# madsjulia/GeostatInversion.jl

Hardware: AMD Instinct MI355X
Metric: randSVD GB/s + top-k singular-value rel-err, n=1e6 rank=256 (higher is better)
Workload: dtype f64

## Files before the change

geostatinversion.jl_amd/csrc/api.cpp:

```cpp
#include <cmath>
#include <cstdlib>
#include <cstring>
#include <memory>
#include <new>
#include <string>
#include <vector>
#include "../../include/gsi_hip.h"
#include "pcga.hpp"
#include "pointcov.hpp"
#include "fftrf_points.hpp"
#include "cg_state.hpp"

using namespace gsi;

struct gsi_ctx {
  Context c;
};
struct gsi_op {
  Operator op;
};
struct gsi_mat {
  gsi_ctx* ctx;
  Buf buf;
  int64_t rows, cols;
// ... 1149 lines not shown
    Backend* be = ctx->c.be.get();
    Buf Wd(be, (size_t)n * l), V(be, (size_t)n * l), S(be, (size_t)l);
    be->upload2d(Wd.p, n, W, n, n, l);
    svd_tall(ctx->c, Wd.p, n, l, -1, V.p, S.p);
    be->download2d(V_out, n, V.p, n, n, l);
    be->download2d(S_out, l, S.p, l, l, 1);
    check_async_errors(ctx->c);
  });
}

int gsi_gemm(gsi_ctx* ctx, int trans, int64_t m, int64_t l, int64_t k, double alpha, const double* A,
             int64_t lda, const double* B, int64_t ldb, double* C, int64_t ldc) {
  return guarded([&] {
    REQUIRE(ctx && A && B && C, "NULL argument");
    REQUIRE(m >= 1 && l >= 1 && k >= 1, "bad shape");
    const int64_t ar = trans ? k : m, ac = trans ? m : k;
    REQUIRE(lda >= ar && ldb >= k && ldc >= m, "leading dimension too small");
    Backend* be = ctx->c.be.get();
    Buf Ad(be, (size_t)ar * ac), Bd(be, (size_t)k * l), Cd(be, (size_t)m * l);
    be->upload2d(Ad.p, ar, A, lda, ar, ac);
    be->upload2d(Bd.p, k, B, ldb, k, l);
    if (trans) be->gemm_tn(m, l, k, alpha, Ad.p, ar, Bd.p, k, 0.0, Cd.p, m);
    else be->gemm_nn(m, l, k, alpha, Ad.p, ar, Bd.p, k, 0.0, Cd.p, m);
    be->download2d(C, ldc, Cd.p, m, m, l);
    check_async_errors(ctx->c);
  });
}

int gsi_gemm_view(gsi_ctx* ctx, int form, int trans, int64_t m, int64_t l, int64_t k, double alpha, double beta,
                  const double* A, int64_t lda, int64_t a_off, const double* B, int64_t ldb, int64_t b_off, double* C,
                  int64_t ldc, int64_t c_off, int64_t m_full, int64_t r0, int64_t* plan_out) {
  return guarded([&] {
    REQUIRE(ctx && A && C && plan_out, "NULL argument");
    REQUIRE(form >= 0 && form <= 3, "gemm_view: form is 0 (gemm), 1 (syrk upper), 2 (trmm upper) or 3 (NN row block)");
    REQUIRE(m >= 1 && l >= 1 && k >= 1, "bad shape");
    REQUIRE(form == 1 || B, "NULL argument");
    REQUIRE(form == 0 || (alpha == 1.0 && beta == 0.0), "gemm_view: forms 1 to 3 compute C = op(A) B (alpha 1, beta 0)");
    REQUIRE(form == 0 || !trans, "gemm_view: trans belongs to form 0");
    REQUIRE(form != 1 || m == l, "gemm_view: form 1 is the l x l product A'A (m == l)");
    REQUIRE(form != 3 || (r0 >= 0 && r0 + m <= m_full), "gemm_view: row block outside the full product");
    const bool tn = trans || form == 1;
    const int64_t ar = (form == 3) ? m_full : (tn ? k : m), ac = tn ? m : k;
    const int64_t crows = (form == 3) ? m_full : m;
    REQUIRE(lda >= ar && ldc >= crows && (form == 1 || ldb >= k), "leading dimension too small");
    REQUIRE(a_off >= 0 && b_off >= 0 && c_off >= 0, "negative offset");
    Backend* be = ctx->c.be.get();
    const size_t na = (size_t)a_off + (size_t)lda * (size_t)ac, nc = (size_t)c_off + (size_t)ldc * (size_t)l;
    const size_t nb = (form == 1) ? 1 : (size_t)b_off + (size_t)ldb * (size_t)l;
    Buf Ad(be, na), Bd(be, nb), Cd(be, nc);
    be->fill_bytes(Ad.p, 0xFF, na);
    be->fill_bytes(Bd.p, 0xFF, nb);
    be->upload2d(Ad.p + a_off, lda, A, ar, ar, ac);
    if (form != 1) be->upload2d(Bd.p + b_off, ldb, B, k, k, l);
    be->upload2d(Cd.p, (int64_t)nc, C, (int64_t)nc, (int64_t)nc, 1);
    be->gemm_view(form, trans != 0, m, l, k, alpha, Ad.p + a_off, lda, Bd.p + b_off, ldb, beta, Cd.p + c_off, ldc, m_full, r0,
                  plan_out);
    be->download2d(C, (int64_t)nc, Cd.p, (int64_t)nc, (int64_t)nc, 1);
    check_async_errors(ctx->c);
  });
}

int gsi_cq_gram_round(gsi_ctx* ctx, int64_t l, int check, const double* gram, double* R, double* X, int32_t* flag_out,
                      int32_t* series_out, double* norm_out) {
  return guarded([&] {
    REQUIRE(ctx && gram && R && X && flag_out && series_out && norm_out, "NULL argument");
    REQUIRE(l >= 1 && l <= 384, "cq_gram_round: 1 <= l <= 384");
    Backend* be = ctx->c.be.get();
    Buf Gd(be, (size_t)l * l), Xd(be, (size_t)l * l);
    be->fill_bytes(Xd.p, 0xFF, (size_t)l * l);
    be->upload2d(Gd.p, l, gram, l, l, l);
    int32_t out2[2] = {0, 0};
    be->cq_gram_round_view(Gd.p, l, Xd.p, check != 0, out2, norm_out);
    be->download2d(R, l, Gd.p, l, l, l);
// ... 665 lines not shown
```

geostatinversion.jl_amd/csrc/backend.hpp:

```cpp
#pragma once
#include <cstddef>
#include <cstdint>
#include <stdexcept>
#include <string>

namespace gsi {

struct Error : std::runtime_error {
  int code;
  Error(int c, const std::string& msg) : std::runtime_error(msg), code(c) {}
};

enum Phase : int {
  PH_GEMM_N = 0, PH_GEMM_T = 1, PH_LU = 2, PH_QR = 3, PH_SVD = 4, PH_SMALL_GEMM = 5,
  PH_COMM = 6, PH_OTHER = 7, PH_COMM_WAIT = 8, PH_COUNT = 9
};

struct FwdProduct {
  int64_t nobs = 0, n = 0, nnz = 0, nseg = 0, maxlen = 0;
  const int64_t* segptr = nullptr;
  const int64_t* rowseg = nullptr;
  const int32_t* colidx = nullptr;
  const double* vals = nullptr;
  const double* w = nullptr;
// ... 20 lines not shown

  virtual double* alloc(size_t count) = 0;
  virtual void release(double* p) = 0;
  virtual int64_t bytes_in_use() const = 0;
  virtual void release_cache() {}
  virtual void upload2d(double* dst, int64_t ldd, const double* host, int64_t ldh, int64_t rows, int64_t cols) = 0;
  virtual void download2d(double* host, int64_t ldh, const double* src, int64_t lds, int64_t rows, int64_t cols) = 0;
  virtual void copy2d(double* dst, int64_t ldd, const double* src, int64_t lds, int64_t rows, int64_t cols) = 0;
  virtual void fill_zero(double* p, size_t count) = 0;
  virtual void sync() = 0;
  virtual int64_t upload_block_rows(int64_t rows, int64_t cols) { (void)cols; return rows; }
  virtual void* upload2d_begin(double* dst, int64_t ldd, const double* host, int64_t ldh, int64_t rows, int64_t cols,
                               int64_t block_rows) {
    (void)block_rows;
    upload2d(dst, ldd, host, ldh, rows, cols);
    return nullptr;
  }
  virtual void pinned_copy_rate(int64_t bytes, double* h2d_gbs, double* d2h_gbs) { (void)bytes; *h2d_gbs = 0.0; *d2h_gbs = 0.0; }
  virtual void upload2d_wait_block(void* handle, int64_t b) { (void)handle; (void)b; }
  virtual void upload2d_end(void* handle) { (void)handle; }

  virtual void gemm_nn(int64_t m, int64_t l, int64_t k, double alpha, const double* A, int64_t lda,
                       const double* B, int64_t ldb, double beta, double* C, int64_t ldc) = 0;
  virtual void gemm_nn_rowblock(int64_t m_full, int64_t r0, int64_t mb, int64_t l, int64_t k, const double* A, int64_t lda,
                                const double* B, int64_t ldb, double* C, int64_t ldc) {
    (void)m_full;
    gemm_nn(mb, l, k, 1.0, A + r0, lda, B, ldb, 0.0, C + r0, ldc);
  }
  virtual void gemm_tn(int64_t m, int64_t l, int64_t k, double alpha, const double* A, int64_t lda,
                       const double* B, int64_t ldb, double beta, double* C, int64_t ldc) = 0;

  virtual void gemm_view(int form, bool trans, int64_t m, int64_t l, int64_t k, double alpha, const double* A, int64_t lda,
                         const double* B, int64_t ldb, double beta, double* C, int64_t ldc, int64_t m_full, int64_t r0,
                         int64_t* plan8) {
    (void)form; (void)trans; (void)m; (void)l; (void)k; (void)alpha; (void)A; (void)lda; (void)B; (void)ldb; (void)beta;
    (void)C; (void)ldc; (void)m_full; (void)r0; (void)plan8;
    throw Error(1 , "gemm_view: not available on this backend");
  }
  virtual void fill_bytes(double* p, int byte, size_t count) {
    (void)p; (void)byte; (void)count;
    throw Error(1 , "fill_bytes: not available on this backend");
  }

  virtual void gemm_nn_gridcov(int64_t m, int64_t l, int64_t k, const double* tab, int64_t nx, int64_t ny,
                               int64_t roff, int64_t koff, const double* B, int64_t ldb, double* C,
                               int64_t ldc) = 0;

  virtual void gemm_nn_pointcov(int64_t m, int64_t l, int64_t k, const double* pts, int d, int kind, double ell,
                                double sigma2, double nugget, int64_t roff, int64_t koff, const double* B, int64_t ldb,
                                double* C, int64_t ldc) = 0;

  virtual void* fftcov_create(const int64_t N[3], double beta, int fftrf) = 0;
  virtual void* fftcov_create_lags(const int64_t N[3], int kind, const double ell[3], double theta, double sigma2,
                                   double nugget, const double* table, const double* table_mirror) {
    (void)N; (void)kind; (void)ell; (void)theta; (void)sigma2; (void)nugget; (void)table; (void)table_mirror;
    throw Error(1 , "fft covariance from a covariance function or table: not supported by this backend");
  }
  virtual void fftcov_destroy(void* plan) = 0;
  virtual void fftcov_apply(void* plan, int64_t l, const double* X, int64_t ldx, double* Y, int64_t ldy) = 0;

  virtual void lu_L(double* Y, int64_t m, int64_t l, int64_t ld, int32_t* ipiv_host_or_null) = 0;
  virtual bool lu_L_keep(double* Y, int64_t m, int64_t l, int64_t ld, int32_t** ipiv_dev) {
    (void)Y; (void)m; (void)l; (void)ld; (void)ipiv_dev;
    return false;
  }
  virtual int lus_block() const = 0;
  virtual void lus_u12_leaf(const double* Yloc, int64_t ld, int64_t row0, int64_t jb, int64_t j0, int w, double* U12) = 0;
  virtual void lus_pending(double* Yloc, int64_t mloc, int64_t ld, int64_t row0, int64_t jb, int64_t j0, int w,
                           const double* U12) = 0;
// ... 293 lines not shown
```

geostatinversion.jl_amd/csrc/gemm_f64.hip:

```cpp
#include <hip/hip_runtime.h>
#include <cstdint>
#include <cstdlib>
#include <type_traits>
#include <algorithm>
#include "hip_common.hpp"
#include "pointcov.hpp"
#include "pointcov_gen.hpp"

namespace gsi { namespace hipk {

#define GSI_GEMM_TILE_COUNTERS_32 1
#include "gemm_f64_kernel.inc.hpp"
void gemm_dispatch_gen1(int nt, dim3 grid, hipStream_t st, int64_t M, int64_t L, int64_t K, const double* A, int64_t lda,
                        const double* B, int64_t ldb, double* C, int64_t ldc, double alpha, double beta, double* slabs,
                        int64_t kchunk, int nchunks_x, int wide, int xmode, int tri, const GenA& gen, int64_t nitems);

__global__ void splitk_reduce_kernel(int64_t M, int64_t L, int nsplit, const double* __restrict__ slabs,
                                     double* __restrict__ C, int64_t ldc, double alpha, double beta) {
  const int64_t total = M * L;
  for (int64_t idx = (int64_t)blockIdx.x * blockDim.x + threadIdx.x; idx < total;
       idx += (int64_t)gridDim.x * blockDim.x) {
    double s = 0.0;
    for (int sp = 0; sp < nsplit; ++sp) s += slabs[(int64_t)sp * total + idx];
    const int64_t r = idx % M, c = idx / M;
// ... 53 lines not shown
  if (M <= 0 || L <= 0) return max_grid <= 0;
  const uint64_t lim = (uint64_t)1 << 32;
  const uint64_t bspan = 8ull * ((uint64_t)(NTMAX * 16) * (uint64_t)ldb + BK);
  const uint64_t aspan = (gen != nullptr) ? 0ull : 8ull * ((uint64_t)(transA ? BMT : BK) * (uint64_t)lda + BMT);
  const bool big = bspan >= lim || aspan >= lim;
  const int64_t tiles = (L + 15) / 16;
  const int ntmax = gemm_chunk_tiles(tri);
  const int64_t nchunks = (tiles + ntmax - 1) / ntmax;
  const int nt = (int)((tiles + nchunks - 1) / nchunks);
  const int64_t rowblocks = (M + BMT - 1) / BMT;
  int64_t active = rowblocks * nchunks;
  if (tri == 1) {
    active = 0;
    for (int64_t rb = 0; rb < rowblocks; ++rb)
      for (int64_t cb = 0; cb < nchunks; ++cb)
        if (cb >= (rb * BMT) / ((int64_t)nt * 16)) ++active;
  }
  const int nsplit = (force_nsplit > 0) ? force_nsplit : ((K > 0) ? gemm_choose_split(active, K) : 1);
  int64_t kchunk = (K + nsplit - 1) / nsplit;
  kchunk = ((kchunk + BK - 1) / BK) * BK;
  if (kchunk == 0) kchunk = BK;
  const int ns_eff = (K > 0) ? (int)((K + kchunk - 1) / kchunk) : 1;
  dim3 grid((unsigned)active, (unsigned)ns_eff, 1);
  double* slabs = (ns_eff > 1) ? ws : nullptr;
  static const int ncus = [] { int dev = 0, n = 256; hipDeviceProp_t pr; if (hipGetDevice(&dev) == hipSuccess && hipGetDeviceProperties(&pr, dev) == hipSuccess) n = pr.multiProcessorCount; return n; }();
  static const bool persist_on = !(getenv("GSI_GEMM_PERSIST") != nullptr && getenv("GSI_GEMM_PERSIST")[0] == '0');
  int64_t nitems = 0;
  const bool a_ok = ((uintptr_t)A & 15) == 0 && (lda & 1) == 0;
  const bool b_ok = ((uintptr_t)B & 15) == 0 && (ldb & 1) == 0;
  const bool irregular_x = a_ok && (!b_ok || L % ((int64_t)nt * 16) != 0);
  const int wide = a_ok ? 1 : 0;
  const int xmode = big ? 2 : (irregular_x ? 1 : 0);
  if (persist_on && gen == nullptr && xmode == 0 && tri == 0 && ns_eff == 1 && (ncus & 7) == 0 && active >= 2 * (int64_t)ncus &&
      K <= 128 * BK) {
    nitems = active;
    grid.x = (unsigned)((max_grid > 0 && max_grid < ncus) ? max_grid : ncus);
  }
  if (max_grid > 0 && nitems == 0 && ((int64_t)grid.x * (int64_t)grid.y > (int64_t)max_grid || ns_eff != 1)) return false;
  if (plan != nullptr) *plan = {nt, nchunks, xmode, wide, ns_eff, nitems > 0 ? 1 : 0, (int64_t)grid.x, active};
  if (query_only) return true;
  const GenA none = {nullptr, 1, 0, 0, 0, 0.0, 0.0, 0.0};
  if (gen != nullptr && gen_mode == 2)
    launch_dispatch<false, 2>(nt, grid, st, M, L, K, A, lda, B, ldb, C, ldc, alpha, beta, slabs, kchunk, (int)nchunks, wide, xmode, tri, *gen, nitems);
  else if (gen != nullptr)
    gemm_dispatch_gen1(nt, grid, st, M, L, K, A, lda, B, ldb, C, ldc, alpha, beta, slabs, kchunk, (int)nchunks, wide, xmode, tri, *gen, nitems);
  else if (transA)
    launch_dispatch<true, 0>(nt, grid, st, M, L, K, A, lda, B, ldb, C, ldc, alpha, beta, slabs, kchunk, (int)nchunks, wide, xmode, tri, none, nitems);
  else
    launch_dispatch<false, 0>(nt, grid, st, M, L, K, A, lda, B, ldb, C, ldc, alpha, beta, slabs, kchunk, (int)nchunks, wide, xmode, tri, none, nitems);
  if (ns_eff > 1) {
    const int64_t total = M * L;
    int blocks = (int)((total + 255) / 256);
    if (blocks > 2048) blocks = 2048;
    hipLaunchKernelGGL(splitk_reduce_kernel, dim3(blocks), dim3(256), 0, st, M, L, ns_eff, slabs, C, ldc,
                       alpha, beta);
  }
  return true;
}

void gemm_splitk_reduce(hipStream_t st, int64_t M, int64_t L, int nsplit, const double* slabs, double* C, int64_t ldc) {
  const int64_t total = M * L;
  int blocks = (int)((total + 255) / 256);
  if (blocks > 2048) blocks = 2048;
  hipLaunchKernelGGL(splitk_reduce_kernel, dim3(blocks), dim3(256), 0, st, M, L, nsplit, slabs, C, ldc, 1.0, 0.0);
}

void gemm_f64(hipStream_t st, bool transA, int64_t M, int64_t L, int64_t K, double alpha, const double* A,
              int64_t lda, const double* B, int64_t ldb, double beta, double* C, int64_t ldc, double* ws, GemmPlan* plan) {
  gemm_launch(st, transA, nullptr, M, L, K, alpha, A, lda, B, ldb, beta, C, ldc, ws, 0, 1, 0, plan);
}

bool gemm_f64_nn_capped(hipStream_t st, int64_t M, int64_t L, int64_t K, const double* A, int64_t lda, const double* B,
                        int64_t ldb, double* C, int64_t ldc, int max_grid, bool query_only, GemmPlan* plan) {
  if (max_grid < 8 || (max_grid & 7) != 0) return false;
  return gemm_launch(st, false, nullptr, M, L, K, 1.0, A, lda, B, ldb, 0.0, C, ldc, nullptr, 0, 1, 1, plan, max_grid, query_only);
}

int gemm_split_for(int64_t M, int64_t L, int64_t K) {
  if (M <= 0 || L <= 0 || K <= 0) return 1;
  const int64_t tiles = (L + 15) / 16, nchunks = (tiles + NTMAX - 1) / NTMAX;
  const int64_t active = ((M + BMT - 1) / BMT) * nchunks;
  return gemm_choose_split(active, K);
// ... 52 lines not shown
```

geostatinversion.jl_amd/csrc/gemm_f64_kernel.inc.hpp:

```cpp
typedef double double4_t __attribute__((ext_vector_type(4)));

constexpr int MT = 2;
constexpr int BMT = 4 * 16 * MT;
constexpr int NTHREADS = 512;
constexpr int BK = 32;
constexpr int BKP = BK + 2;
constexpr int BMP = BMT + 16;
constexpr int NTMAX = 10;
constexpr int NSETS = 2;
constexpr int A_PAIRS = BMT * BK / (2 * NTHREADS);
constexpr int KSTEP_NN = 2 * NTHREADS / BMT;
constexpr int RSTEP = 2 * NTHREADS / BK;
static_assert(A_PAIRS * 2 * NTHREADS == BMT * BK, "tile does not divide over the threads");

struct GenA {
  const double* t2;
  int32_t ny;
  int32_t kind;
  int64_t roff;
  int64_t koff;
  double inv_ell2, sigma2, nugget;
  int32_t dim;
};

// ... 200 lines not shown
        }
        return;
      }
#pragma unroll
      for (int it = 0; it < B_PAIRS; ++it)
        if (!B_RAGGED || b_c + RSTEP * it < NT * 16)
          b_reg[set][it] = *reinterpret_cast<const double2*>(Bb + (b_off0 + (off_t)it * b_step));
      return;
    }
    if constexpr (GEN == 0) {
#pragma unroll
    for (int it = 0; it < A_PAIRS; ++it) {
      const char* p = Ab + (a_off0 + (off_t)it * a_step);
      const int64_t r = TRANS_A ? r0 + a_r + RSTEP * it : r0 + a_r;
      const int64_t k = TRANS_A ? k0 + a_k : k0 + a_k + KSTEP_NN * it;
      const bool ok0 = (r < M && k < kend);
      const bool ok1 = TRANS_A ? (r < M && k + 1 < kend) : (r + 1 < M && k < kend);
      a_reg[set][it].x = ok0 ? *reinterpret_cast<const double*>(p) : 0.0;
      a_reg[set][it].y = ok1 ? *reinterpret_cast<const double*>(p + 8) : 0.0;
    }
    }
#pragma unroll
    for (int it = 0; it < B_PAIRS; ++it) {
      const char* p = Bb + (b_off0 + (off_t)it * b_step);
      const int cl = b_c + RSTEP * it;
      const int64_t c = c0 + cl;
      const int64_t k = k0 + b_k;
      const bool okc = (cl < NT * 16) && (c < L);
      b_reg[set][it].x = (okc && k < kend) ? *reinterpret_cast<const double*>(p) : 0.0;
      b_reg[set][it].y = (okc && k + 1 < kend) ? *reinterpret_cast<const double*>(p + 8) : 0.0;
    }
  };

  auto stage = [&](int buf, auto SET, int64_t k0) __attribute__((always_inline)) {
    constexpr int set = decltype(SET)::value;
    double* a_s = smem + LDS0 + buf * BUF_ELEMS;
    double* b_s = a_s + A_ELEMS;
    (void)k0;
    if constexpr (GEN == 2) {
      const int kw = __builtin_amdgcn_readfirstlane(a_k);
      const int64_t row_first = gen.roff + r0;
      const int krem = (kend - k0 < BK) ? (int)(kend - k0) : BK;
#pragma unroll
      for (int it = 0; it < A_PAIRS; ++it) {
        const int64_t kc = k0 + kw + KSTEP_NN * it;
        const bool okk = kw + KSTEP_NN * it < krem;
        const int64_t gj = gen.koff + (okk ? kc : kbeg);
        const int64_t gju = ((int64_t)__builtin_amdgcn_readfirstlane((int)(gj >> 32)) << 32) |
                            (uint32_t)__builtin_amdgcn_readfirstlane((int)(gj & 0xffffffff));
        const double qx = A[4 * gju], qy = A[4 * gju + 1];
        double dx = p0x - qx, dy = p0y - qy;
        double s0 = fma(dx, dx, dy * dy);
        dx = p1x - qx; dy = p1y - qy;
        double s1 = fma(dx, dx, dy * dy);
        const int fl = gen_flags(gq.flags);
        if (fl & 1) {
          const double qz = A[4 * gju + 2];
          const double dz0 = p0z - qz, dz1 = p1z - qz;
          s0 = fma(dz0, dz0, s0); s1 = fma(dz1, dz1, s1);
        }
        double2 pr;
        gen_point_pair(gq, fl, s0, s1, gtab, pr.x, pr.y);
        const int rel = (int)(gju - row_first);
        if ((unsigned)rel < (unsigned)BMT) {
          pr.x += (a_r == rel) ? gen.nugget : 0.0;
          pr.y += (a_r + 1 == rel) ? gen.nugget : 0.0;
// ... 13 lines not shown
#pragma unroll
    for (int it = 0; it < B_PAIRS; ++it)
      if (!B_RAGGED || b_c + RSTEP * it < NT * 16)
        *reinterpret_cast<double2*>(b_s + (b_c + RSTEP * it) * BKP + b_k) = b_reg[set][it];
  };

  double fa[MT], fan[MT];
  double fb[NTW];
  const int t0 = ch * NTW;
  const int ntw = (NT - t0 < NTW) ? ((NT - t0 > 0) ? NT - t0 : 0) : NTW;
  auto a_frag = [&](int buf, int s, int h) -> double {
    const double* a_s = smem + LDS0 + buf * BUF_ELEMS;
    return TRANS_A ? a_s[(16 * MT * rg + 16 * h + jl) * BKP + 4 * s + kk]
                   : a_s[(4 * s + kk) * BMP + 16 * MT * rg + 16 * h + jl];
  };
  auto b_frag = [&](int buf, int s, int t) -> double {
    const double* b_s = smem + LDS0 + buf * BUF_ELEMS + A_ELEMS;
    return b_s[(16 * (t0 + t) + jl) * BKP + 4 * s + kk];
  };

  using Set0 = std::integral_constant<int, 0>;
  using Set1 = std::integral_constant<int, 1>;
#if GSI_GEMM_TILE_COUNTERS_32
  auto do_tile = [&](int t, auto PAR) __attribute__((always_inline)) {
#else
  auto do_tile = [&](int64_t t, auto PAR) __attribute__((always_inline)) {
#endif
    constexpr int cur = decltype(PAR)::value;
    using NextSet = std::integral_constant<int, (NSETS == 2) ? (cur ^ 1) : 0>;
    auto chores = [&]() __attribute__((always_inline)) {
      __builtin_amdgcn_s_setprio(0);
#if GSI_GEMM_TILE_COUNTERS_32
      if (t + 1 < ntiles) stage(cur ^ 1, NextSet{}, kbeg + (int64_t)(t + 1) * BK);
      if (t + 1 + NSETS < ntiles) prefetch(t + 1 + NSETS, NextSet{});
#else
      if (t + 1 < ntiles) stage(cur ^ 1, NextSet{}, kbeg + (t + 1) * BK);
      if (t + 1 + NSETS < ntiles) prefetch(kbeg + (t + 1 + NSETS) * BK, NextSet{});
#endif
      __builtin_amdgcn_s_setprio(1);
    };
#pragma unroll
    for (int s = 0; s < BK / 4; ++s) {
      if (s == 1 && ch == 0) chores();
      if (s == 1 + BK / 8 && ch != 0) chores();
      const bool last = (s + 1 == BK / 4);
      if (last) __syncthreads();
      const int nbuf = last ? (cur ^ 1) : cur;
      const int ns = last ? 0 : s + 1;
      const bool more = !last || (t + 1 < ntiles);
      if (more) {
#pragma unroll
        for (int h = 0; h < MT; ++h) fan[h] = a_frag(nbuf, ns, h);
      }
#pragma unroll
      for (int tt = 0; tt < NTW; ++tt) {
        if ((NT % 2 == 0) || tt < ntw) {
#pragma unroll
          for (int h = 0; h < MT; ++h)
            acc[h][tt] = __builtin_amdgcn_mfma_f64_16x16x4f64(fb[tt], fa[h], acc[h][tt], 0, 0, 0);
          if (more) fb[tt] = b_frag(nbuf, ns, tt);
        }
      }
#pragma unroll
      for (int h = 0; h < MT; ++h) fa[h] = fan[h];
    }
  };

  int64_t item = blockIdx.x;
  bool primed = false;
  for (;;) {
    if (ntiles > 0) {
      if (!primed) {
#if GSI_GEMM_TILE_COUNTERS_32
        prefetch(0, Set0{});
        if (NSETS == 2 && ntiles > 1) prefetch(1, Set1{});
#else
        prefetch(kbeg, Set0{});
        if (NSETS == 2 && ntiles > 1) prefetch(kbeg + BK, Set1{});
#endif
      }
      stage(0, Set0{}, kbeg);
#if GSI_GEMM_TILE_COUNTERS_32
      if (ntiles > NSETS) prefetch(NSETS, Set0{});
#else
      if (ntiles > NSETS) prefetch(kbeg + NSETS * BK, Set0{});
#endif
      __syncthreads();
#pragma unroll
      for (int h = 0; h < MT; ++h) fa[h] = a_frag(0, 0, h);
#pragma unroll
      for (int t = 0; t < NTW; ++t)
        if ((NT % 2 == 0) || t < ntw) fb[t] = b_frag(0, 0, t);
#if GSI_GEMM_TILE_COUNTERS_32
      int t = 0;
#else
      int64_t t = 0;
#endif
      for (; t + 1 < ntiles; t += 2) {
        do_tile(t, Set0{});
        do_tile(t + 1, Set1{});
      }
      if (t < ntiles) do_tile(t, Set0{});
    }
    const int64_t er0 = r0, ec0 = c0;
    bool more = false;
    if constexpr (CANP) {
      if (persist && item + (int64_t)gridDim.x < nitems) {
        more = true;
        item += gridDim.x;
        __syncthreads();
        locate(item);
        setup_item();
        if (ntiles > 0) {
#if GSI_GEMM_TILE_COUNTERS_32
          prefetch(0, Set0{});
          if (NSETS == 2 && ntiles > 1) prefetch(1, Set1{});
#else
          prefetch(kbeg, Set0{});
          if (NSETS == 2 && ntiles > 1) prefetch(kbeg + BK, Set1{});
#endif
        }
        primed = true;
      }
    }

#pragma unroll
    for (int h = 0; h < MT; ++h) {
      const int64_t row = er0 + 16 * MT * rg + 16 * h + jl;
      if (row < M) {
        double* W = (slabs != nullptr) ? slabs + (int64_t)split * M * L : nullptr;
#pragma unroll
        for (int t = 0; t < NTW; ++t) {
          if ((NT % 2 == 0) || t < ntw) {
#pragma unroll
            for (int reg = 0; reg < 4; ++reg) {
              const int64_t col = ec0 + 16 * (t0 + t) + kk + 4 * reg;
              if (col < L) {
                if (W != nullptr) {
                  W[row + col * M] = acc[h][t][reg];
                } else {
                  double v = alpha * acc[h][t][reg];
                  if (beta != 0.0) v += beta * C[row + col * ldc];
                  C[row + col * ldc] = v;
                }
              }
            }
          }
        }
      }
    }
    if (!more) break;
#pragma unroll
    for (int h = 0; h < MT; ++h)
#pragma unroll
// ... 44 lines not shown
```

geostatinversion.jl_amd/csrc/hip_backend_impl.hpp:

```cpp
#pragma once
#include <map>
#include <memory>
#include <mutex>
#include <set>
#include <string>
#include <vector>
#include "hip_backend.hpp"
#include "hip_common.hpp"
#include "host_staging.hpp"
#include "fftrf_points.hpp"

namespace gsi {

struct DevBuf {
  void* p = nullptr;
  size_t bytes = 0;
  bool pooled = false;
};

struct Carve {
  size_t total = 0;
  static constexpr size_t up8(size_t x) { return (x + 7) & ~(size_t)7; }
  size_t take(size_t count) { const size_t o = total; total += up8(count); return o; }
  size_t packed(size_t count) { const size_t o = total; total += count; return o; }
// ... 66 lines not shown
  void* upload2d_begin(double* dst, int64_t ldd, const double* host, int64_t ldh, int64_t rows, int64_t cols,
                       int64_t block_rows) override;
  void upload2d_wait_block(void* handle, int64_t b) override;
  void upload2d_end(void* handle) override;
  void pinned_copy_rate(int64_t bytes, double* h2d_gbs, double* d2h_gbs) override;
  void copy2d(double* dst, int64_t ldd, const double* src, int64_t lds, int64_t rows, int64_t cols) override;
  void fill_zero(double* p, size_t count) override;
  void fill_bytes(double* p, int byte, size_t count) override;
  void sync() override;
  void forgive_lost_coresidency() override;
  bool retryable_failure() override;
  int take_error(std::string* msg) override;
  void profile(bool on) override { prof_ = on; }
  void phase_begin(Phase p) override;
  void phase_end(Phase) override { phase_end_counted(true); }
  void phase_end_more(Phase) override { phase_end_counted(false); }
  void phase_reset() override;
  void phase_times(double* ms, int64_t* counts) override;
  void counters(int64_t* out4) override;
  int64_t lu_timeouts() override { return n_lu_timeouts_; }
  int64_t svd_cap_hits() override { return n_svd_cap_hits_; }
  int64_t lowrank_tail_overlaps() override { return n_tail_overlaps_; }
  int64_t lowrank_tail_series_rounds() override { return n_tail_series_rounds_; }
  void set_ranks_sharing_device(int n) override { ranks_sharing_device_ = n; }

  void gemm_nn(int64_t m, int64_t l, int64_t k, double alpha, const double* A, int64_t lda, const double* B,
               int64_t ldb, double beta, double* C, int64_t ldc) override;
  void gemm_nn_rowblock(int64_t m_full, int64_t r0, int64_t mb, int64_t l, int64_t k, const double* A, int64_t lda,
                        const double* B, int64_t ldb, double* C, int64_t ldc) override;
  void gemm_tn(int64_t m, int64_t l, int64_t k, double alpha, const double* A, int64_t lda, const double* B,
               int64_t ldb, double beta, double* C, int64_t ldc) override;
  void gemm_view(int form, bool trans, int64_t m, int64_t l, int64_t k, double alpha, const double* A, int64_t lda,
                 const double* B, int64_t ldb, double beta, double* C, int64_t ldc, int64_t m_full, int64_t r0,
                 int64_t* plan8) override;
  void gemm_nn_gridcov(int64_t m, int64_t l, int64_t k, const double* tab, int64_t nx, int64_t ny, int64_t roff,
                       int64_t koff, const double* B, int64_t ldb, double* C, int64_t ldc) override;
  void gemm_nn_pointcov(int64_t m, int64_t l, int64_t k, const double* pts, int d, int kind, double ell, double sigma2,
                        double nugget, int64_t roff, int64_t koff, const double* B, int64_t ldb, double* C,
                        int64_t ldc) override;
  void* fftcov_create(const int64_t N[3], double beta, int fftrf) override;
  void* fftcov_create_lags(const int64_t N[3], int kind, const double ell[3], double theta, double sigma2, double nugget,
                           const double* table, const double* table_mirror) override;
  void fftcov_destroy(void* plan) override;
  void fftcov_apply(void* plan, int64_t l, const double* X, int64_t ldx, double* Y, int64_t ldy) override;
  void center_rows(double* S, int64_t n, int64_t N, int64_t ld) override;
  void randn(double* p, size_t count, uint64_t seed) override;
  void fill_gridcov(double* A, int64_t lda, int64_t nx, int64_t ny, double ell, int kind, int64_t row0,
                    int64_t mloc) override;
  void fill_lowrank_samples(double* S, int64_t ld, int64_t nloc, int64_t N, int64_t row0, uint64_t seed,
                            double decay) override;
  void fftrf_fields(double* dst, int64_t ldd, int64_t row0, int64_t nloc, int64_t nf, int ndims, const int64_t* N, double k0,
                    double dk, double beta, const double* phi, int64_t ldphi, uint64_t seed, int64_t field0) override;
  void fftrf_fields_at(double* dst, int64_t ldd, int64_t nf, int ndims, const int64_t* N, double k0, double dk, double beta,
                       const double* phi, int64_t ldphi, uint64_t seed, int64_t field0, const FftrfPointsPlan& plan) override;
  void fftrf_interpolate(double* dst, int64_t ldd, int64_t nf, const double* grid, int64_t ldg,
                         const FftrfPointsPlan& plan) override;
  void* points_at_create(const FftrfPointsPlan& plan, int64_t info[4]) override;
  void points_at_destroy(void* at) override;
  void points_at_gather(void* at, double* dst, int64_t ldd, int64_t nf, const double* grid, int64_t ldg) override;
  void points_at_spread(void* at, double* grid, int64_t ldg, int64_t nf, const double* src, int64_t lds) override;

  void* gridcov_sampler_create(int ndims, const int64_t N[3], const int64_t M[3], int kind, const double ell[3], double theta,
                               double sigma2, double nugget, double neg_tol, double info[4]) override;
  void gridcov_sampler_destroy(void* plan) override;
  void gridcov_sampler_spectrum(void* plan, double* lam_host) override;
  void gridcov_sampler_fields(void* plan, double* dst, int64_t ldd, int64_t row0, int64_t nloc, int64_t nf, const double* eps,
                              int64_t ldeps, uint64_t seed, int64_t field0) override;
// ... 213 lines not shown
```

geostatinversion.jl_amd/csrc/hip_backend_products.hip:

```cpp
#include <algorithm>
#include <cmath>
#include <cstdlib>
#include <cstring>
#include "hip_backend_impl.hpp"
#include "interp_adjoint_plan.hpp"

namespace gsi {

void HipBackend::fits_ws(const char* who, const char* form, size_t need, const GemmWs& ws, int64_t m, int64_t l, int64_t k) {
  if (need <= ws.doubles) return;
  throw Error(GSI_ERR_INTERNAL, std::string(who) + ": the " + form + " product " + std::to_string(m) + " x " + std::to_string(l) +
                                    " (K = " + std::to_string(k) + ") needs a workspace of " + std::to_string(need) +
                                    " doubles and was given " + std::to_string(ws.doubles));
}
void HipBackend::gemm(const char* who, const GemmWs& ws, bool trans, int64_t m, int64_t l, int64_t k, double alpha,
                      const double* A, int64_t lda, const double* B, int64_t ldb, double beta, double* C, int64_t ldc,
                      hipk::GemmPlan* plan) {
  fits_ws(who, trans ? "A'B" : "AB", hipk::gemm_workspace_doubles(m, l, k), ws, m, l, k);
  hipk::gemm_f64(st_, trans, m, l, k, alpha, A, lda, B, ldb, beta, C, ldc, ws.p, plan);
}
void HipBackend::gemm_rowblock(const char* who, const GemmWs& ws, int64_t m_full, int64_t r0, int64_t mb, int64_t l, int64_t k,
                               const double* A, int64_t lda, const double* B, int64_t ldb, double* C, int64_t ldc,
                               hipk::GemmPlan* plan) {
  fits_ws(who, "row-block", hipk::gemm_rowblock_workspace_doubles(m_full, mb, l, k), ws, mb, l, k);
// ... 3 lines not shown
                                 double* C, int64_t ldc, hipk::GemmPlan* plan) {
  fits_ws(who, "A'A", hipk::gemm_syrk_workspace_doubles(l, k), ws, l, l, k);
  hipk::gemm_f64_syrk_upper(st_, l, k, A, lda, C, ldc, ws.p, plan);
}
void HipBackend::gemm_trmm_upper(const char* who, const GemmWs& ws, int64_t m, int64_t l, int64_t k, const double* A,
                                 int64_t lda, const double* B, int64_t ldb, double* C, int64_t ldc, hipk::GemmPlan* plan) {
  fits_ws(who, "A triu(B)", hipk::gemm_workspace_doubles(m, l, k), ws, m, l, k);
  hipk::gemm_f64_trmm_upper(st_, m, l, k, A, lda, B, ldb, C, ldc, ws.p, plan);
}

void HipBackend::gemm_nn(int64_t m, int64_t l, int64_t k, double alpha, const double* A, int64_t lda, const double* B,
                         int64_t ldb, double beta, double* C, int64_t ldc) {
  bind();
  const GemmWs ws = gemm_ws(hipk::gemm_workspace_doubles(m, l, k));
  gemm("gemm_nn", ws, false, m, l, k, alpha, A, lda, B, ldb, beta, C, ldc);
  check_launch("gemm_nn");
}
void HipBackend::gemm_nn_rowblock(int64_t m_full, int64_t r0, int64_t mb, int64_t l, int64_t k, const double* A, int64_t lda,
                                  const double* B, int64_t ldb, double* C, int64_t ldc) {
  bind();
  const GemmWs ws = gemm_ws(hipk::gemm_rowblock_workspace_doubles(m_full, mb, l, k));
  gemm_rowblock("gemm_nn_rowblock", ws, m_full, r0, mb, l, k, A, lda, B, ldb, C, ldc);
  check_launch("gemm_nn_rowblock");
}
void HipBackend::gemm_tn(int64_t m, int64_t l, int64_t k, double alpha, const double* A, int64_t lda, const double* B,
                         int64_t ldb, double beta, double* C, int64_t ldc) {
  bind();
  const GemmWs ws = gemm_ws(hipk::gemm_workspace_doubles(m, l, k));
  gemm("gemm_tn", ws, true, m, l, k, alpha, A, lda, B, ldb, beta, C, ldc);
  check_launch("gemm_tn");
}
void HipBackend::gemm_view(int form, bool trans, int64_t m, int64_t l, int64_t k, double alpha, const double* A, int64_t lda,
                           const double* B, int64_t ldb, double beta, double* C, int64_t ldc, int64_t m_full, int64_t r0,
                           int64_t* plan8) {
  bind();
  hipk::GemmPlan p = {0, 0, 0, 0, 0, 0, 0, 0};
  if (form == 0) {
    const GemmWs ws = gemm_ws(hipk::gemm_workspace_doubles(m, l, k));
    gemm("gemm_view", ws, trans, m, l, k, alpha, A, lda, B, ldb, beta, C, ldc, &p);
  } else if (form == 1) {
    const GemmWs ws = gemm_ws(hipk::gemm_syrk_workspace_doubles(l, k));
    gemm_syrk_upper("gemm_view", ws, l, k, A, lda, C, ldc, &p);
  } else if (form == 2) {
    const GemmWs ws = gemm_ws(hipk::gemm_workspace_doubles(m, l, k));
    gemm_trmm_upper("gemm_view", ws, m, l, k, A, lda, B, ldb, C, ldc, &p);
  } else {
    const GemmWs ws = gemm_ws(hipk::gemm_rowblock_workspace_doubles(m_full, m, l, k));
    gemm_rowblock("gemm_view", ws, m_full, r0, m, l, k, A, lda, B, ldb, C, ldc, &p);
  }
  check_launch("gemm_view");
  const int64_t out[8] = {p.nt, p.nchunks, p.xmode, p.wide, p.nsplit, p.persistent, p.grid_x, p.active};
  for (int i = 0; i < 8; ++i) plan8[i] = out[i];
}
void HipBackend::gemm_nn_gridcov(int64_t m, int64_t l, int64_t k, const double* tab, int64_t nx, int64_t ny, int64_t roff,
                                 int64_t koff, const double* B, int64_t ldb, double* C, int64_t ldc) {
  bind();
  double* ws = gemm_ws(hipk::gemm_workspace_doubles(m, l, k)).p;
  hipk::gemm_f64_gridcov(st_, m, l, k, tab, nx, ny, roff, koff, B, ldb, C, ldc, ws);
  check_launch("gemm_nn_gridcov");
}

void HipBackend::gemm_nn_pointcov(int64_t m, int64_t l, int64_t k, const double* pts, int d, int kind, double ell, double sigma2,
                                  double nugget, int64_t roff, int64_t koff, const double* B, int64_t ldb, double* C,
                                  int64_t ldc) {
  bind();
  if (m <= 0 || l <= 0 || k <= 0) return;
  const int64_t npts = std::max(roff + m, koff + k);
  Scratch p4(this, (size_t)4 * npts);
  hipk::pointcov_pad_points(st_, pts, d, npts, hipk::pointcov_point_scale(kind, 1.0 / ell), p4.p);
  double* ws = gemm_ws(hipk::gemm_pointcov_workspace_doubles(m, l, k)).p;
  Scratch xpack(this);
  const size_t xdoubles = hipk::gemm_pointcov_pack_doubles(m, l, k);
  if (xdoubles > 0) xpack.try_alloc(xdoubles);
  hipk::gemm_f64_pointcov(st_, m, l, k, p4.p, npts, d, kind, sigma2, nugget, roff, koff, B, ldb, C, ldc, ws, xpack.p);
  check_launch("gemm_nn_pointcov (in-loader generator)");
}

struct HipBackend::FftCov {
  int64_t N[3], M[3]; Scratch lam, W; int nb_max;
  explicit FftCov(HipBackend* be) : lam(be), W(be) {}
};
std::unique_ptr<HipBackend::FftCov> HipBackend::fftcov_new_plan(const int64_t N[3], int fftrf, bool* reembed, int* dims) {
  std::unique_ptr<FftCov> p(new FftCov(this));
  int64_t Mtot = 1;
  int d = 0;
// ... 284 lines not shown
```

geostatinversion.jl_amd/csrc/hip_common.hpp:

```cpp
#pragma once
#include <hip/hip_runtime.h>
#include <atomic>
#include <cstdint>
#include <cstddef>
#include "pointcov.hpp"

namespace gsi { struct FwdProduct; }

namespace gsi { namespace hipk {

inline bool first_use_on_this_device(std::atomic<uint64_t>& mask) {
  int dev = 0;
  if (hipGetDevice(&dev) != hipSuccess || dev < 0 || dev > 63) return true;
  const uint64_t bit = (uint64_t)1 << dev;
  return (mask.fetch_or(bit, std::memory_order_acq_rel) & bit) == 0;
}

struct GemmPlan { int64_t nt, nchunks, xmode, wide, nsplit, persistent, grid_x, active; };
size_t gemm_workspace_doubles(int64_t M, int64_t L, int64_t K);
void gemm_f64(hipStream_t st, bool transA, int64_t M, int64_t L, int64_t K, double alpha, const double* A,
              int64_t lda, const double* B, int64_t ldb, double beta, double* C, int64_t ldc, double* ws,
              GemmPlan* plan = nullptr);
bool gemm_f64_nn_capped(hipStream_t st, int64_t M, int64_t L, int64_t K, const double* A, int64_t lda, const double* B,
                        int64_t ldb, double* C, int64_t ldc, int max_grid, bool query_only = false, GemmPlan* plan = nullptr);
size_t gemm_rowblock_workspace_doubles(int64_t M_full, int64_t mb, int64_t L, int64_t K);
void gemm_f64_nn_rowblock(hipStream_t st, int64_t M_full, int64_t r0, int64_t mb, int64_t L, int64_t K, const double* A,
                          int64_t lda, const double* B, int64_t ldb, double* C, int64_t ldc, double* ws,
                          GemmPlan* plan = nullptr);
size_t gemm_syrk_workspace_doubles(int64_t l, int64_t m);
size_t syrk_upper_workspace_doubles(int64_t l, int64_t m);
bool syrk_full_from_upper(hipStream_t st, int64_t l, int64_t m, const double* Y, int64_t ld, double* G, int64_t ldg, double* ws);
bool trmm_upper_tall(hipStream_t st, int64_t m, int64_t l, const double* A, int64_t lda, const double* X, int64_t ldx, double* C,
                     int64_t ldc);
void gemm_f64_syrk_upper(hipStream_t st, int64_t l, int64_t m, const double* A, int64_t lda, double* C, int64_t ldc,
                         double* ws, GemmPlan* plan = nullptr);
void gemm_f64_trmm_upper(hipStream_t st, int64_t M, int64_t L, int64_t K, const double* A, int64_t lda, const double* B,
                         int64_t ldb, double* C, int64_t ldc, double* ws, GemmPlan* plan = nullptr);
void gemm_f64_gridcov(hipStream_t st, int64_t M, int64_t L, int64_t K, const double* tab, int64_t nx, int64_t ny,
                      int64_t roff, int64_t koff, const double* B, int64_t ldb, double* C, int64_t ldc, double* ws);

void gemm_f64_pointcov(hipStream_t st, int64_t M, int64_t L, int64_t K, const double* pts4, int64_t npts, int d, int kind,
                       double sigma2, double nugget, int64_t roff, int64_t koff, const double* B, int64_t ldb, double* C,
                       int64_t ldc, double* ws, double* xpack);
double pointcov_point_scale(int kind, double inv_ell);
bool gemm_f64_pointcov_wide(hipStream_t st, int64_t M, int64_t L, int64_t K, const double* pts4, int64_t npts, int d, int kind,
                            double sigma2, double nugget, int64_t roff, int64_t koff, const double* B, int64_t ldb, double* C,
                            int64_t ldc, double* ws, double* xpack);
size_t gemm_pointcov_workspace_doubles(int64_t M, int64_t L, int64_t K);
size_t gemm_pointcov_pack_doubles(int64_t M, int64_t L, int64_t K);
int gemm_choose_split(int64_t nwg, int64_t K);
void gemm_splitk_reduce(hipStream_t st, int64_t M, int64_t L, int nsplit, const double* slabs, double* C, int64_t ldc);
// ... 273 lines not shown
```

geostatinversion.jl_amd/randmatfact.py:

```python
import ctypes as C

import numpy as np

from . import _lib as L
from .context import Operator, dense_operator, default_context

_rng = np.random.default_rng()


def seed(s):
    global _rng
    _rng = np.random.default_rng(s)


def randn(*shape):
    if len(shape) == 1:
        return _rng.standard_normal(shape[0])
    n, l = shape
    return np.asfortranarray(_rng.standard_normal((l, n)).T)


def _as_operator(A, ctx=None):
    if isinstance(A, Operator):
        return A, False
# ... 248 lines not shown
    m, l = Yf.shape
    Q = np.empty((m, l), order="F")
    R = np.empty((l, l), order="F")
    L.check(ctx.lib.gsi_qr_thinQ(ctx.h, L.dptr(Yf), m, l, L.dptr(Q), L.dptr(R)), ctx.lib)
    return (Q, R) if return_R else Q


def svd_tall(W, *, ctx=None):
    ctx = ctx or default_context()
    Wf = L.fmat(W, "W")
    n, l = Wf.shape
    V = np.empty((n, l), order="F")
    S = np.empty(l)
    L.check(ctx.lib.gsi_svd_tall(ctx.h, L.dptr(Wf), n, l, L.dptr(V), S.ctypes.data_as(L.c_dp)), ctx.lib)
    return S, V


def gemm(A, B, *, trans=False, alpha=1.0, ctx=None):
    ctx = ctx or default_context()
    Af, Bf = L.fmat(A, "A"), L.fmat(B, "B")
    if trans:
        k, m = Af.shape
    else:
        m, k = Af.shape
    if Bf.shape[0] != k:
        raise ValueError("dimension mismatch")
    l = Bf.shape[1]
    Cm = np.empty((m, l), order="F")
    L.check(ctx.lib.gsi_gemm(ctx.h, int(trans), m, l, k, float(alpha), L.dptr(Af), Af.shape[0], L.dptr(Bf), k,
                             L.dptr(Cm), m), ctx.lib)
    return Cm


GEMM_PLAN_FIELDS = ("nt", "nchunks", "xmode", "wide", "nsplit", "persistent", "grid_x", "active")


def gemm_view(A, B, C_image, *, m, l, k, form=0, trans=False, alpha=1.0, beta=0.0, lda, a_off=0, ldb=0, b_off=0, ldc,
              c_off=0, m_full=0, r0=0, ctx=None):
    ctx = ctx or default_context()
    Af = L.fmat(A, "A")
    Bf = None if B is None else L.fmat(B, "B")
    img = np.array(C_image, dtype=np.float64).reshape(-1)
    if img.size != c_off + ldc * l:
        raise ValueError("C_image must hold c_off + ldc * l doubles")
    ar, ac = (m_full, k) if form == 3 else ((k, m) if (trans or form == 1) else (m, k))
    if Af.shape != (ar, ac) or (Bf is not None and Bf.shape != (k, l)):
        raise ValueError("dimension mismatch")
    plan = np.zeros(8, dtype=np.int64)
    L.check(ctx.lib.gsi_gemm_view(ctx.h, int(form), int(bool(trans)), m, l, k, float(alpha), float(beta), L.dptr(Af), lda,
                                  a_off, None if Bf is None else L.dptr(Bf), ldb, b_off, L.dptr(img), ldc, c_off, m_full, r0,
                                  plan.ctypes.data_as(C.POINTER(L.c_i64))), ctx.lib)
    return img, dict(zip(GEMM_PLAN_FIELDS, (int(v) for v in plan)))


def cq_gram_round(gram, *, check=True, ctx=None):
    ctx = ctx or default_context()
    Gf = L.fmat(gram, "gram")
    l = Gf.shape[0]
    if Gf.shape != (l, l):
        raise ValueError("gram must be square")
    Rm, Xm = np.empty((l, l), order="F"), np.empty((l, l), order="F")
    flag, series, norm = C.c_int32(0), C.c_int32(0), C.c_double(0.0)
    L.check(ctx.lib.gsi_cq_gram_round(ctx.h, l, int(bool(check)), L.dptr(Gf), L.dptr(Rm), L.dptr(Xm), C.byref(flag),
                                      C.byref(series), C.byref(norm)), ctx.lib)
    return Rm, Xm, int(flag.value), int(series.value), float(norm.value)
```

Measured before the change: 1772.

## Prefetch next persistent work item's first tiles during current item's tail

In the persistent NN GEMM kernel, each workgroup now peeks at its next work item and, once the current item has no more of its own tiles to prefetch, uses the free prefetch slots to load the next item's first K tiles. This hides the restart latency between items that previously began with a cold prefetch. It adds packed tile coordinates (limited to fewer than 256 column chunks and 2^23 row blocks), extra register state and an env switch to disable the path. A capped-grid gemm_view form and a carry field in the plan are added for testing.

```diff
diff --git a/geostatinversion.jl_amd/csrc/api.cpp b/geostatinversion.jl_amd/csrc/api.cpp
--- a/geostatinversion.jl_amd/csrc/api.cpp
+++ b/geostatinversion.jl_amd/csrc/api.cpp
@@ -1205,13 +1205,14 @@
                   int64_t ldc, int64_t c_off, int64_t m_full, int64_t r0, int64_t* plan_out) {
   return guarded([&] {
     REQUIRE(ctx && A && C && plan_out, "NULL argument");
-    REQUIRE(form >= 0 && form <= 3, "gemm_view: form is 0 (gemm), 1 (syrk upper), 2 (trmm upper) or 3 (NN row block)");
+    REQUIRE(form >= 0 && form <= 4, "gemm_view: form is 0 (gemm), 1 (syrk upper), 2 (trmm upper), 3 (NN row block) or 4 (NN under a grid cap)");
     REQUIRE(m >= 1 && l >= 1 && k >= 1, "bad shape");
     REQUIRE(form == 1 || B, "NULL argument");
-    REQUIRE(form == 0 || (alpha == 1.0 && beta == 0.0), "gemm_view: forms 1 to 3 compute C = op(A) B (alpha 1, beta 0)");
+    REQUIRE(form == 0 || (alpha == 1.0 && beta == 0.0), "gemm_view: forms 1 to 4 compute C = op(A) B (alpha 1, beta 0)");
     REQUIRE(form == 0 || !trans, "gemm_view: trans belongs to form 0");
     REQUIRE(form != 1 || m == l, "gemm_view: form 1 is the l x l product A'A (m == l)");
     REQUIRE(form != 3 || (r0 >= 0 && r0 + m <= m_full), "gemm_view: row block outside the full product");
+    REQUIRE(form != 4 || (r0 >= 8 && r0 % 8 == 0 && r0 < (int64_t)1 << 30), "gemm_view: form 4 takes the grid cap in r0, a multiple of 8");
     const bool tn = trans || form == 1;
     const int64_t ar = (form == 3) ? m_full : (tn ? k : m), ac = tn ? m : k;
     const int64_t crows = (form == 3) ? m_full : m;
diff --git a/geostatinversion.jl_amd/csrc/backend.hpp b/geostatinversion.jl_amd/csrc/backend.hpp
--- a/geostatinversion.jl_amd/csrc/backend.hpp
+++ b/geostatinversion.jl_amd/csrc/backend.hpp
@@ -76,9 +76,9 @@
 
   virtual void gemm_view(int form, bool trans, int64_t m, int64_t l, int64_t k, double alpha, const double* A, int64_t lda,
                          const double* B, int64_t ldb, double beta, double* C, int64_t ldc, int64_t m_full, int64_t r0,
-                         int64_t* plan8) {
+                         int64_t* plan9) {
     (void)form; (void)trans; (void)m; (void)l; (void)k; (void)alpha; (void)A; (void)lda; (void)B; (void)ldb; (void)beta;
-    (void)C; (void)ldc; (void)m_full; (void)r0; (void)plan8;
+    (void)C; (void)ldc; (void)m_full; (void)r0; (void)plan9;
     throw Error(1 , "gemm_view: not available on this backend");
   }
   virtual void fill_bytes(double* p, int byte, size_t count) {
diff --git a/geostatinversion.jl_amd/csrc/gemm_f64.hip b/geostatinversion.jl_amd/csrc/gemm_f64.hip
--- a/geostatinversion.jl_amd/csrc/gemm_f64.hip
+++ b/geostatinversion.jl_amd/csrc/gemm_f64.hip
@@ -109,12 +109,14 @@
   const int wide = a_ok ? 1 : 0;
   const int xmode = big ? 2 : (irregular_x ? 1 : 0);
   if (persist_on && gen == nullptr && xmode == 0 && tri == 0 && ns_eff == 1 && (ncus & 7) == 0 && active >= 2 * (int64_t)ncus &&
-      K <= 128 * BK) {
+      K <= 128 * BK && nchunks <= 256 && rowblocks < ((int64_t)1 << 23)) {
     nitems = active;
     grid.x = (unsigned)((max_grid > 0 && max_grid < ncus) ? max_grid : ncus);
   }
+  static const bool carry_on = !(getenv("GSI_GEMM_CARRY") != nullptr && getenv("GSI_GEMM_CARRY")[0] == '0');
+  const bool carry = carry_on && nitems > 0 && !transA && wide != 0 && (K + BK - 1) / BK > NSETS;
   if (max_grid > 0 && nitems == 0 && ((int64_t)grid.x * (int64_t)grid.y > (int64_t)max_grid || ns_eff != 1)) return false;
-  if (plan != nullptr) *plan = {nt, nchunks, xmode, wide, ns_eff, nitems > 0 ? 1 : 0, (int64_t)grid.x, active};
+  if (plan != nullptr) *plan = {nt, nchunks, xmode, wide, ns_eff, nitems > 0 ? 1 : 0, (int64_t)grid.x, active, carry ? 1 : 0};
   if (query_only) return true;
   const GenA none = {nullptr, 1, 0, 0, 0, 0.0, 0.0, 0.0};
   if (gen != nullptr && gen_mode == 2)
@@ -124,7 +126,7 @@
   else if (transA)
     launch_dispatch<true, 0>(nt, grid, st, M, L, K, A, lda, B, ldb, C, ldc, alpha, beta, slabs, kchunk, (int)nchunks, wide, xmode, tri, none, nitems);
   else
-    launch_dispatch<false, 0>(nt, grid, st, M, L, K, A, lda, B, ldb, C, ldc, alpha, beta, slabs, kchunk, (int)nchunks, wide, xmode, tri, none, nitems);
+    launch_dispatch<false, 0>(nt, grid, st, M, L, K, A, lda, B, ldb, C, ldc, alpha, beta, slabs, kchunk, (int)nchunks, wide | (carry ? 2 : 0), xmode, tri, none, nitems);
   if (ns_eff > 1) {
     const int64_t total = M * L;
     int blocks = (int)((total + 255) / 256);
diff --git a/geostatinversion.jl_amd/csrc/gemm_f64_kernel.inc.hpp b/geostatinversion.jl_amd/csrc/gemm_f64_kernel.inc.hpp
--- a/geostatinversion.jl_amd/csrc/gemm_f64_kernel.inc.hpp
+++ b/geostatinversion.jl_amd/csrc/gemm_f64_kernel.inc.hpp
@@ -256,6 +256,26 @@
     }
   };
 
+#if GSI_GEMM_TILE_COUNTERS_32
+  constexpr bool CANC = CANP && !TRANS_A;
+  const bool carry = CANC && persist && (wide & 2) != 0 && ntiles > NSETS;
+  int64_t item = blockIdx.x;
+  int32_t nxt = INT32_MIN;
+  auto peek = [&]() __attribute__((always_inline)) {
+    nxt = INT32_MIN;
+    if (item + (int64_t)gridDim.x < nitems) {
+      const int64_t sr0 = r0, sc0 = c0;
+      locate(item + (int64_t)gridDim.x);
+      const bool early = carry && (r0 + BMT <= M) && (c0 + NT * 16 <= L);
+      nxt = (int32_t)(((uint32_t)(r0 / BMT) << 8) | (uint32_t)(c0 / (NT * 16)) | (early ? 0u : 0x80000000u));
+      r0 = sr0; c0 = sc0;
+    }
+  };
+  auto nxt_r0 = [&]() -> int64_t { return (int64_t)(((uint32_t)nxt & 0x7fffffffu) >> 8) * BMT; };
+  auto nxt_c0 = [&]() -> int64_t { return (int64_t)((uint32_t)nxt & 0xffu) * (NT * 16); };
+  if constexpr (CANC) { if (persist) peek(); }
+#endif
+
   auto stage = [&](int buf, auto SET, int64_t k0) __attribute__((always_inline)) {
     constexpr int set = decltype(SET)::value;
     double* a_s = smem + LDS0 + buf * BUF_ELEMS;
@@ -335,7 +355,25 @@
       __builtin_amdgcn_s_setprio(0);
 #if GSI_GEMM_TILE_COUNTERS_32
       if (t + 1 < ntiles) stage(cur ^ 1, NextSet{}, kbeg + (int64_t)(t + 1) * BK);
-      if (t + 1 + NSETS < ntiles) prefetch(t + 1 + NSETS, NextSet{});
+      if constexpr (CANC) {
+        const bool mine = t + 1 + NSETS < ntiles;
+        if (mine || (nxt >= 0 && t + 1 < ntiles)) {
+          const char* const sa = Abase;
+          const char* const sb = Bbase;
+          const bool sf = wg_full;
+          int tt = t + 1 + NSETS;
+          if (!mine) {
+            tt = cur ^ 1;
+            Abase = reinterpret_cast<const char*>(TRANS_A ? A + nxt_r0() * lda : A + nxt_r0());
+            Bbase = reinterpret_cast<const char*>(B + nxt_c0() * ldb);
+            wg_full = true;
+          }
+          prefetch(tt, NextSet{});
+          Abase = sa; Bbase = sb; wg_full = sf;
+        }
+      } else {
+        if (t + 1 + NSETS < ntiles) prefetch(t + 1 + NSETS, NextSet{});
+      }
 #else
       if (t + 1 < ntiles) stage(cur ^ 1, NextSet{}, kbeg + (t + 1) * BK);
       if (t + 1 + NSETS < ntiles) prefetch(kbeg + (t + 1 + NSETS) * BK, NextSet{});
@@ -369,7 +407,9 @@
     }
   };
 
+#if !GSI_GEMM_TILE_COUNTERS_32
   int64_t item = blockIdx.x;
+#endif
   bool primed = false;
   for (;;) {
     if (ntiles > 0) {
@@ -412,17 +452,28 @@
         more = true;
         item += gridDim.x;
         __syncthreads();
+#if GSI_GEMM_TILE_COUNTERS_32
+        bool early = false;
+        if constexpr (CANC) {
+          early = nxt >= 0;
+          r0 = nxt_r0(); c0 = nxt_c0();
+        } else {
+          locate(item);
+        }
+        setup_item();
+        if (ntiles > 0 && !early) {
+          prefetch(0, Set0{});
+          if (NSETS == 2 && ntiles > 1) prefetch(1, Set1{});
+        }
+        if constexpr (CANC) peek();
+#else
         locate(item);
         setup_item();
         if (ntiles > 0) {
-#if GSI_GEMM_TILE_COUNTERS_32
-          prefetch(0, Set0{});
-          if (NSETS == 2 && ntiles > 1) prefetch(1, Set1{});
-#else
           prefetch(kbeg, Set0{});
           if (NSETS == 2 && ntiles > 1) prefetch(kbeg + BK, Set1{});
-#endif
-        }
+        }
+#endif
         primed = true;
       }
     }
diff --git a/geostatinversion.jl_amd/csrc/hip_backend_impl.hpp b/geostatinversion.jl_amd/csrc/hip_backend_impl.hpp
--- a/geostatinversion.jl_amd/csrc/hip_backend_impl.hpp
+++ b/geostatinversion.jl_amd/csrc/hip_backend_impl.hpp
@@ -122,7 +122,7 @@
                int64_t ldb, double beta, double* C, int64_t ldc) override;
   void gemm_view(int form, bool trans, int64_t m, int64_t l, int64_t k, double alpha, const double* A, int64_t lda,
                  const double* B, int64_t ldb, double beta, double* C, int64_t ldc, int64_t m_full, int64_t r0,
-                 int64_t* plan8) override;
+                 int64_t* plan9) override;
   void gemm_nn_gridcov(int64_t m, int64_t l, int64_t k, const double* tab, int64_t nx, int64_t ny, int64_t roff,
                        int64_t koff, const double* B, int64_t ldb, double* C, int64_t ldc) override;
   void gemm_nn_pointcov(int64_t m, int64_t l, int64_t k, const double* pts, int d, int kind, double ell, double sigma2,
diff --git a/geostatinversion.jl_amd/csrc/hip_backend_products.hip b/geostatinversion.jl_amd/csrc/hip_backend_products.hip
--- a/geostatinversion.jl_amd/csrc/hip_backend_products.hip
+++ b/geostatinversion.jl_amd/csrc/hip_backend_products.hip
@@ -59,7 +59,7 @@
 }
 void HipBackend::gemm_view(int form, bool trans, int64_t m, int64_t l, int64_t k, double alpha, const double* A, int64_t lda,
                            const double* B, int64_t ldb, double beta, double* C, int64_t ldc, int64_t m_full, int64_t r0,
-                           int64_t* plan8) {
+                           int64_t* plan9) {
   bind();
   hipk::GemmPlan p = {0, 0, 0, 0, 0, 0, 0, 0};
   if (form == 0) {
@@ -71,13 +71,16 @@
   } else if (form == 2) {
     const GemmWs ws = gemm_ws(hipk::gemm_workspace_doubles(m, l, k));
     gemm_trmm_upper("gemm_view", ws, m, l, k, A, lda, B, ldb, C, ldc, &p);
-  } else {
+  } else if (form == 3) {
     const GemmWs ws = gemm_ws(hipk::gemm_rowblock_workspace_doubles(m_full, m, l, k));
     gemm_rowblock("gemm_view", ws, m_full, r0, m, l, k, A, lda, B, ldb, C, ldc, &p);
+  } else {
+    if (!hipk::gemm_f64_nn_capped(st_, m, l, k, A, lda, B, ldb, C, ldc, (int)r0, false, &p))
+      throw Error(GSI_ERR_ARG, "gemm_view: the capped product does not apply to this shape under a cap of " + std::to_string(r0));
   }
   check_launch("gemm_view");
-  const int64_t out[8] = {p.nt, p.nchunks, p.xmode, p.wide, p.nsplit, p.persistent, p.grid_x, p.active};
-  for (int i = 0; i < 8; ++i) plan8[i] = out[i];
+  const int64_t out[9] = {p.nt, p.nchunks, p.xmode, p.wide, p.nsplit, p.persistent, p.grid_x, p.active, p.carry};
+  for (int i = 0; i < 9; ++i) plan9[i] = out[i];
 }
 void HipBackend::gemm_nn_gridcov(int64_t m, int64_t l, int64_t k, const double* tab, int64_t nx, int64_t ny, int64_t roff,
                                  int64_t koff, const double* B, int64_t ldb, double* C, int64_t ldc) {
diff --git a/geostatinversion.jl_amd/csrc/hip_common.hpp b/geostatinversion.jl_amd/csrc/hip_common.hpp
--- a/geostatinversion.jl_amd/csrc/hip_common.hpp
+++ b/geostatinversion.jl_amd/csrc/hip_common.hpp
@@ -16,7 +16,7 @@
   return (mask.fetch_or(bit, std::memory_order_acq_rel) & bit) == 0;
 }
 
-struct GemmPlan { int64_t nt, nchunks, xmode, wide, nsplit, persistent, grid_x, active; };
+struct GemmPlan { int64_t nt, nchunks, xmode, wide, nsplit, persistent, grid_x, active, carry; };
 size_t gemm_workspace_doubles(int64_t M, int64_t L, int64_t K);
 void gemm_f64(hipStream_t st, bool transA, int64_t M, int64_t L, int64_t K, double alpha, const double* A,
               int64_t lda, const double* B, int64_t ldb, double beta, double* C, int64_t ldc, double* ws,
diff --git a/geostatinversion.jl_amd/randmatfact.py b/geostatinversion.jl_amd/randmatfact.py
--- a/geostatinversion.jl_amd/randmatfact.py
+++ b/geostatinversion.jl_amd/randmatfact.py
@@ -304,7 +304,7 @@
     return Cm
 
 
-GEMM_PLAN_FIELDS = ("nt", "nchunks", "xmode", "wide", "nsplit", "persistent", "grid_x", "active")
+GEMM_PLAN_FIELDS = ("nt", "nchunks", "xmode", "wide", "nsplit", "persistent", "grid_x", "active", "carry")
 
 
 def gemm_view(A, B, C_image, *, m, l, k, form=0, trans=False, alpha=1.0, beta=0.0, lda, a_off=0, ldb=0, b_off=0, ldc,
@@ -318,7 +318,7 @@
     ar, ac = (m_full, k) if form == 3 else ((k, m) if (trans or form == 1) else (m, k))
     if Af.shape != (ar, ac) or (Bf is not None and Bf.shape != (k, l)):
         raise ValueError("dimension mismatch")
-    plan = np.zeros(8, dtype=np.int64)
+    plan = np.zeros(len(GEMM_PLAN_FIELDS), dtype=np.int64)
     L.check(ctx.lib.gsi_gemm_view(ctx.h, int(form), int(bool(trans)), m, l, k, float(alpha), float(beta), L.dptr(Af), lda,
                                   a_off, None if Bf is None else L.dptr(Bf), ldb, b_off, L.dptr(img), ldc, c_off, m_full, r0,
                                   plan.ctypes.data_as(C.POINTER(L.c_i64))), ctx.lib)
```

Result: no change. 1783, median of 6 (+0.6%).
